# dog-qiuqiu/Yolo-FastestV2

Measured on NVIDIA B200. Metric: images/sec 352x352 fwd+decode+NMS, higher is better.
Workload: dtype f32

## Files before the change

yolo-fastestv2_b200/csrc/eng3.cuh:

```cuda
#pragma once
#include "common.cuh"
#include "tc.cuh"

namespace yfv2 {
namespace eng3 {

using namespace tc;

struct BPipe {
    uint64_t empty[2];
    uint64_t dfull;
    uint32_t arrivals[2];
};
struct BGrp {
    uint32_t tcol, tlane;
    BPipe* pipe;
    uint32_t chunk;
    uint32_t dparity;
    int gtid;
};

__device__ __forceinline__ uint32_t atom_inc_acq_rel(uint32_t* addr) {
    uint32_t old;
    asm volatile("atom.acq_rel.cta.shared::cta.add.u32 %0, [%1], 1;" : "=r"(old) : "r"(smem_u32(addr)) : "memory");
    return old;
}
__device__ __forceinline__ void publish_async() { asm volatile("fence.proxy.async.shared::cta;" ::: "memory"); }
__device__ __forceinline__ void tmem_ld16v(uint32_t taddr, float* v) {
    uint32_t r[16];
    asm volatile("tcgen05.ld.sync.aligned.32x32b.x16.b32 {%0, %1, %2, %3, %4, %5, %6, %7, %8, %9, %10, %11, %12, %13, %14, %15}, [%16];"
                 : "=r"(r[0]), "=r"(r[1]), "=r"(r[2]), "=r"(r[3]), "=r"(r[4]), "=r"(r[5]), "=r"(r[6]), "=r"(r[7]), "=r"(r[8]),
                   "=r"(r[9]), "=r"(r[10]), "=r"(r[11]), "=r"(r[12]), "=r"(r[13]), "=r"(r[14]), "=r"(r[15])
                 : "r"(taddr) : "memory");
#pragma unroll
    for (int i = 0; i < 16; ++i) v[i] = __uint_as_float(r[i]);
}


template <int NB>
__device__ __forceinline__ void st_acquire(BGrp& g) {
    const uint32_t buf = g.chunk % NB, use = g.chunk / NB;
    if (use > 0) mbar_wait(&g.pipe->empty[buf], (use - 1) & 1u);
    fence_after_sync();
}
template <int KC, int NB>
__device__ __forceinline__ void st_store(const BGrp& g, const float* a) {
    const uint32_t col = g.tlane + (g.chunk % NB) * (2 * KC);
#pragma unroll
    for (int j = 0; j < KC; j += 8) {
        uint32_t hi[8], lo[8];
#pragma unroll
        for (int i = 0; i < 8; ++i) {
            hi[i] = __float_as_uint(a[j + i]) & 0xFFFFE000u;
            lo[i] = __float_as_uint(a[j + i] - __uint_as_float(hi[i]));
        }
        tmem_st8(col + j, hi);
        tmem_st8(col + KC + j, lo);
    }
}
template <int KP, int NP, int KC, int NB>
__device__ __forceinline__ void st_hand_off(BGrp& g, int c, uint32_t b_hi, uint32_t b_lo, uint32_t dcol, bool last) {
    wait_st();
    fence_before_sync();
    __syncwarp();
    if ((threadIdx.x & 31) == 0) {
        const uint32_t buf = g.chunk % NB;
        const uint32_t old = atom_inc_acq_rel(&g.pipe->arrivals[buf]);
        if ((old & 3u) == 3u) {
            fence_after_sync();
            constexpr uint32_t idesc = make_idesc_tf32(128, NP);
            constexpr uint32_t LBO = 128, SBO = (KP / 4) * 128;
            const uint32_t a_hi = g.tcol + buf * (2 * KC), a_lo = a_hi + KC, d = g.tcol + dcol;
#pragma unroll
            for (int s = 0; s < KC / 8; ++s) {
                const int ks = c * (KC / 8) + s;
                const uint64_t bh = make_b_desc(b_hi + ks * 256, LBO, SBO);
                const uint64_t bl = make_b_desc(b_lo + ks * 256, LBO, SBO);
                mma_tf32_ts(d, a_lo + 8 * s, bh, idesc, ks > 0 ? 1u : 0u);
                mma_tf32_ts(d, a_hi + 8 * s, bl, idesc, 1u);
                mma_tf32_ts(d, a_hi + 8 * s, bh, idesc, 1u);
            }
            mma_commit(&g.pipe->empty[buf]);
            if (last) mma_commit(&g.pipe->dfull);
        }
    }
    __syncwarp();
    ++g.chunk;
}
__device__ __forceinline__ void st_wait_d(BGrp& g) {
    mbar_wait(&g.pipe->dfull, g.dparity);
    g.dparity ^= 1u;
    fence_after_sync();
}

}
}
```

yolo-fastestv2_b200/csrc/k_blk.cu:

```cuda
#include <cstdlib>

#include "eng3.cuh"

namespace yfv2 {
namespace {

using namespace tc;
using namespace eng3;

constexpr int kMaxChain = 7;
constexpr int kMaxK = 48;

template <int KC, int NB>
__device__ __forceinline__ void acquire_buf(BGrp& g) {
    const uint32_t buf = g.chunk % NB, use = g.chunk / NB;
    if (use > 0) mbar_wait(&g.pipe->empty[buf], (use - 1) & 1u);
    fence_after_sync();
}
template <int KC, int NB, int KCS = KC>
__device__ __forceinline__ void store_a(const BGrp& g, int tile, const float* a, int koff = 0) {
    const uint32_t col = g.tlane + (g.chunk % NB) * (4 * KC) + tile * (2 * KC) + koff;
#pragma unroll
    for (int j = 0; j < KCS; j += 8) {
        uint32_t hi[8], lo[8];
#pragma unroll
        for (int i = 0; i < 8; ++i) {
            hi[i] = __float_as_uint(a[j + i]) & 0xFFFFE000u;
            lo[i] = __float_as_uint(a[j + i] - __uint_as_float(hi[i]));
        }
        tmem_st8(col + j, hi);
        tmem_st8(col + KC + j, lo);
    }
}
template <int KP, int NP, int KC, int NB, int SIB = 1>
__device__ __forceinline__ void hand_off(BGrp& g, int c, uint32_t b_hi, uint32_t b_lo) {
    wait_st();
    fence_before_sync();
    __syncwarp();
    if ((threadIdx.x & 31) == 0) {
        const uint32_t buf = g.chunk % NB;
        const uint32_t old = atom_inc_acq_rel(&g.pipe->arrivals[buf]);
        if ((old & (4u * SIB - 1u)) == 4u * SIB - 1u) {
            fence_after_sync();
            constexpr uint32_t idesc = make_idesc_tf32(128, NP);
            constexpr uint32_t LBO = 128, SBO = (KP / 4) * 128;
#pragma unroll
            for (int t = 0; t < 2; ++t) {
                const uint32_t a_hi = g.tcol + buf * (4 * KC) + t * (2 * KC), a_lo = a_hi + KC;
                const uint32_t d = g.tcol + NB * 4 * KC + t * NP;
#pragma unroll
                for (int s = 0; s < KC / 8; ++s) {
                    const int ks = c * (KC / 8) + s;
                    const uint64_t bh = make_b_desc(b_hi + ks * 256, LBO, SBO);
                    const uint64_t bl = make_b_desc(b_lo + ks * 256, LBO, SBO);
                    mma_tf32_ts(d, a_lo + 8 * s, bh, idesc, ks > 0 ? 1u : 0u);
                    mma_tf32_ts(d, a_hi + 8 * s, bl, idesc, 1u);
                    mma_tf32_ts(d, a_hi + 8 * s, bh, idesc, 1u);
                }
            }
            mma_commit(&g.pipe->empty[buf]);
            if (c == KP / KC - 1) mma_commit(&g.pipe->dfull);
        }
    }
    __syncwarp();
    ++g.chunk;
}
template <int KC, int NB>
__device__ __forceinline__ void wait_d(BGrp& g) {
    mbar_wait(&g.pipe->dfull, g.dparity);
    g.dparity ^= 1u;
    fence_after_sync();
}
template <int NP, int KC, int NB>
__device__ __forceinline__ void load_d(const BGrp& g, int tile, float* d) {
#pragma unroll
    for (int n0 = 0; n0 < NP; n0 += 16) tmem_ld16v(g.tlane + NB * 4 * KC + tile * NP + n0, d + n0);
    wait_ld();
}

struct S1cArgs {
    Planes P;
    const float* w1[kMaxChain];
    const float* w2[kMaxChain];
    const float* wdw[kMaxChain];
    uint32_t in_off[kMaxChain][kMaxK];
    uint32_t out_off[kMaxChain][kMaxK];
    int nblk;
    int N, TR, bandsPerImg;
    int wbufs;
};

template <int K, int NP>
struct S1Smem {
    static constexpr int WFL = 2 * NP * K + 2 * NP;
    static constexpr int WSET = 2 * WFL + K * 12;
};
__host__ __device__ constexpr int t_half_floats(int TR, int W) { return ((TR + 3) / 2) * W + 2; }

template <int K, int NP, int G, int KC, int NB, int SIB = 1>
__global__ void __launch_bounds__(G * 128 * SIB, 1)
s1c_kernel(const __grid_constant__ S1cArgs p) {
    pdl_trigger();
    constexpr int KP = K;
    constexpr int COLS = NB * 4 * KC + 2 * NP;
    constexpr int KCS = KC / SIB, NT = G * 128 * SIB;
    static_assert(G * COLS <= 512 && K % KC == 0 && KCS % 8 == 0 && NP % 16 == 0 && K <= kMaxK && (SIB == 1 || SIB == 2), "shape");
    using L = S1Smem<K, NP>;
    extern __shared__ __align__(128) float smem[];
    __shared__ __align__(8) BPipe pipes[G];
    __shared__ __align__(8) uint64_t wbar[2];
    __shared__ uint32_t tmem_slot;
    float* sW = smem;
    float* T = sW + (size_t)p.wbufs * L::WSET;
    const int H = p.P.H, W = p.P.W;
    const int TH = t_half_floats(p.TR, W);
    const int TP = 2 * TH;
    const int warp = threadIdx.x >> 5;
    const int items = p.N * p.bandsPerImg;
    const int my_items = ((int)blockIdx.x < items) ? (items - 1 - (int)blockIdx.x) / (int)gridDim.x + 1 : 0;
    const int total_sets = p.nblk > 1 ? my_items * p.nblk : min(my_items, 1);

    auto load_wset = [&](int seq) {
        const int b = seq % p.nblk, buf = seq % p.wbufs;
        float* dst = sW + (size_t)buf * L::WSET;
        mbar_expect_tx(&wbar[buf], (uint32_t)(L::WSET * sizeof(float)));
        bulk_g2s(dst, p.w1[b], L::WFL * sizeof(float), &wbar[buf]);
        bulk_g2s(dst + L::WFL, p.w2[b], L::WFL * sizeof(float), &wbar[buf]);
        bulk_g2s(dst + 2 * L::WFL, p.wdw[b], K * 12 * sizeof(float), &wbar[buf]);
    };

    if (threadIdx.x == 32) {
        mbar_init(&wbar[0], 1); mbar_init(&wbar[1], 1);
        for (int i = 0; i < G; ++i) {
            mbar_init(&pipes[i].empty[0], 1); mbar_init(&pipes[i].empty[1], 1); mbar_init(&pipes[i].dfull, 1);
            pipes[i].arrivals[0] = 0; pipes[i].arrivals[1] = 0;
        }
        fence_mbar_init();
        if (total_sets > 0) load_wset(0);
        if (total_sets > 1 && p.wbufs > 1) load_wset(1);
    }
    if (warp == 0) tmem_alloc(&tmem_slot, 512);
    for (int i = threadIdx.x; i < K * TP; i += NT) T[i] = 0.f;
    fence_before_sync();
    __syncthreads();
    fence_after_sync();
    BGrp g;
    const int grp = threadIdx.x / (128 * SIB);
    const int sub = SIB == 1 ? 0 : (warp >> 2) & 1;
    const int koff = sub * KCS;
    g.tcol = tmem_slot + grp * COLS;
    g.tlane = g.tcol + ((uint32_t)(32 * (warp & 3)) << 16);
    g.pipe = &pipes[grp];
    g.chunk = 0; g.dparity = 0;
    g.gtid = threadIdx.x & 127;
    pdl_wait();

    int seq = 0;
    for (int item = blockIdx.x; item < items; item += gridDim.x) {
        const int n = item / p.bandsPerImg;
        const int r0 = (item - n * p.bandsPerImg) * p.TR;
        const int rows = min(p.TR, H - r0);
        float* const img = p.P.base + (long long)n * p.P.sN + p.P.org;
        const int tr_lo = r0 == 0 ? 1 : 0, tr_hi = (r0 + rows == H) ? rows : rows + 1;
        if (p.bandsPerImg > 1) {
            if (r0 == 0) for (int i = threadIdx.x; i < K * W; i += NT) { const int k = i / W; T[k * TP + 1 + (i - k * W)] = 0.f; }
            if (r0 + rows == H) {
                const int tr = rows + 1;
                const int o = (tr & 1) * TH + 1 + (tr >> 1) * W;
                for (int i = threadIdx.x; i < K * W; i += NT) { const int k = i / W; T[k * TP + o + (i - k * W)] = 0.f; }
            }
            __syncthreads();
        }
        for (int b = 0; b < p.nblk; ++b) {
            const int wb = seq % p.wbufs;
            const float* sB1 = sW + (size_t)wb * L::WSET;
            const float* sB2 = sB1 + L::WFL;
            const float* sDW = sB2 + L::WFL;
            mbar_wait(&wbar[wb], (uint32_t)(seq / p.wbufs) & 1u);
            const uint32_t b1_hi = smem_u32(sB1), b1_lo = smem_u32(sB1 + NP * KP);
            const uint32_t b2_hi = smem_u32(sB2), b2_lo = smem_u32(sB2 + NP * KP);
            const float* aff1 = sB1 + 2 * NP * KP;
            const float* aff2 = sB2 + 2 * NP * KP;
            const uint32_t* ioff = p.in_off[b];
            const uint32_t* ooff = p.out_off[b];
            const int i_lo = (tr_lo + 1) >> 1, i_hi = (tr_hi + 1) >> 1;
            const int nbp = (i_hi - i_lo + 1) * W;
            for (int tile = grp; tile * 128 < nbp; tile += G) {
                const int q = tile * 128 + g.gtid;
                const bool inb = q < nbp;
                const int qc = inb ? q : 0;
                const int ii = qc / W, x = qc - ii * W;
                const int i = i_lo + ii;
                const int tr0 = 2 * i - 1, tr1 = 2 * i;
                const bool v0 = inb && tr0 >= tr_lo, v1 = inb && tr1 <= tr_hi;
                const int gr0 = r0 - 1 + (tr0 >= tr_lo ? tr0 : tr1), gr1 = r0 - 1 + (tr1 <= tr_hi ? tr1 : tr0);
                const float* ip0 = img + gr0 * p.P.Ws + x;
                const float* ip1 = img + gr1 * p.P.Ws + x;
                float v[2][2 * KCS];
#pragma unroll
                for (int j = 0; j < KCS; ++j) { v[0][j] = __ldcg(ip0 + ioff[koff + j]); v[0][KCS + j] = __ldcg(ip1 + ioff[koff + j]); }
#pragma unroll
                for (int c = 0; c < K / KC; ++c) {
                    if (c + 1 < K / KC) {
#pragma unroll
                        for (int j = 0; j < KCS; ++j) {
                            v[(c + 1) & 1][j] = __ldcg(ip0 + ioff[(c + 1) * KC + koff + j]);
                            v[(c + 1) & 1][KCS + j] = __ldcg(ip1 + ioff[(c + 1) * KC + koff + j]);
                        }
                    }
                    acquire_buf<KC, NB>(g);
                    store_a<KC, NB, KCS>(g, 0, v[c & 1], koff);
                    store_a<KC, NB, KCS>(g, 1, v[c & 1] + KCS, koff);
                    hand_off<KP, NP, KC, NB, SIB>(g, c, b1_hi, b1_lo);
                }
                wait_d<KC, NB>(g);
                float* te = T + 1 + i * W + x;
                float* to = T + TH + 1 + (i - 1) * W + x;
#pragma unroll
                for (int t = 0; t < 2; ++t) {
                    if (SIB == 2 && t != sub) continue;
                    float d[NP];
                    load_d<NP, KC, NB>(g, t, d);
                    if (t == 0 ? v0 : v1) {
                        float* tp = t == 0 ? to : te;
#pragma unroll
                        for (int n4 = 0; n4 < K; n4 += 4) {
                            const float4 sc = *reinterpret_cast<const float4*>(aff1 + n4);
                            const float4 sh = *reinterpret_cast<const float4*>(aff1 + NP + n4);
                            tp[(n4 + 0) * TP] = fmaxf(fmaf(d[n4 + 0], sc.x, sh.x), 0.f);
                            tp[(n4 + 1) * TP] = fmaxf(fmaf(d[n4 + 1], sc.y, sh.y), 0.f);
                            tp[(n4 + 2) * TP] = fmaxf(fmaf(d[n4 + 2], sc.z, sh.z), 0.f);
                            tp[(n4 + 3) * TP] = fmaxf(fmaf(d[n4 + 3], sc.w, sh.w), 0.f);
                        }
                    }
                }
            }
            __syncthreads();
            const int ncp = ((rows + 1) >> 1) * W;
            for (int tile = grp; tile * 128 < ncp; tile += G) {
                const int q = tile * 128 + g.gtid;
                const bool inb = q < ncp;
                const int qc = inb ? q : 0;
                const int j = qc / W, ox = qc - j * W;
                const bool v0 = inb, v1 = inb && 2 * j + 1 < rows;
                const float mL = ox > 0 ? 1.f : 0.f, mR = ox < W - 1 ? 1.f : 0.f;
                const float* te = T + qc;
                const float* to = te + TH;
#pragma unroll 1
                for (int c = 0; c < K / KC; ++c) {
                    float a0[KCS], a1[KCS];
                    const float* e = te + (c * KC + koff) * TP;
                    const float* o = to + (c * KC + koff) * TP;
                    const float* wk = sDW + (c * KC + koff) * 12;
#pragma unroll
                    for (int jj = 0; jj < KCS; ++jj) {
                        const float4 wa = *reinterpret_cast<const float4*>(wk);
                        const float4 wb4 = *reinterpret_cast<const float4*>(wk + 4);
                        const float4 wc = *reinterpret_cast<const float4*>(wk + 8);
                        const float r0l = e[0], r0c = e[1], r0r = e[2];
                        const float r1l = o[0], r1c = o[1], r1r = o[2];
                        const float r2l = e[W], r2c = e[W + 1], r2r = e[W + 2];
                        const float r3l = o[W], r3c = o[W + 1], r3r = o[W + 2];
                        float cl0 = wa.x * r0l; cl0 = fmaf(wa.w, r1l, cl0); cl0 = fmaf(wb4.z, r2l, cl0);
                        float cc0 = wa.y * r0c; cc0 = fmaf(wb4.x, r1c, cc0); cc0 = fmaf(wb4.w, r2c, cc0);
                        float cr0 = wa.z * r0r; cr0 = fmaf(wb4.y, r1r, cr0); cr0 = fmaf(wc.x, r2r, cr0);
                        float cl1 = wa.x * r1l; cl1 = fmaf(wa.w, r2l, cl1); cl1 = fmaf(wb4.z, r3l, cl1);
                        float cc1 = wa.y * r1c; cc1 = fmaf(wb4.x, r2c, cc1); cc1 = fmaf(wb4.w, r3c, cc1);
                        float cr1 = wa.z * r1r; cr1 = fmaf(wb4.y, r2r, cr1); cr1 = fmaf(wc.x, r3r, cr1);
                        const float d0 = fmaf(mR, cr0, fmaf(mL, cl0, cc0));
                        const float d1 = fmaf(mR, cr1, fmaf(mL, cl1, cc1));
                        a0[jj] = fmaf(d0, wc.y, wc.z);
                        a1[jj] = fmaf(d1, wc.y, wc.z);
                        e += TP; o += TP; wk += 12;
                    }
                    acquire_buf<KC, NB>(g);
                    store_a<KC, NB, KCS>(g, 0, a0, koff);
                    store_a<KC, NB, KCS>(g, 1, a1, koff);
                    hand_off<KP, NP, KC, NB, SIB>(g, c, b2_hi, b2_lo);
                }
                wait_d<KC, NB>(g);
                float* op = img + (r0 + 2 * j) * p.P.Ws + ox;
#pragma unroll
                for (int t = 0; t < 2; ++t) {
                    if (SIB == 2 && t != sub) continue;
                    float d[NP];
                    load_d<NP, KC, NB>(g, t, d);
                    if (t == 0 ? v0 : v1) {
                        float* o2 = op + t * p.P.Ws;
#pragma unroll
                        for (int n4 = 0; n4 < K; n4 += 4) {
                            const float4 sc = *reinterpret_cast<const float4*>(aff2 + n4);
                            const float4 sh = *reinterpret_cast<const float4*>(aff2 + NP + n4);
                            o2[ooff[n4 + 0]] = fmaxf(fmaf(d[n4 + 0], sc.x, sh.x), 0.f);
                            o2[ooff[n4 + 1]] = fmaxf(fmaf(d[n4 + 1], sc.y, sh.y), 0.f);
                            o2[ooff[n4 + 2]] = fmaxf(fmaf(d[n4 + 2], sc.z, sh.z), 0.f);
                            o2[ooff[n4 + 3]] = fmaxf(fmaf(d[n4 + 3], sc.w, sh.w), 0.f);
                        }
                    }
                }
            }
            __syncthreads();
            if (p.nblk > 1) {
                if (threadIdx.x == 32 && seq + p.wbufs < total_sets) {
                    publish_async();
                    load_wset(seq + p.wbufs);
                }
                ++seq;
            }
        }
    }
    fence_before_sync();
    __syncthreads();
    if (warp == 0) tmem_dealloc(tmem_slot, 512);
}

template <int S>
__device__ __forceinline__ float dw3(const float* __restrict__ r0, const float* __restrict__ r1, const float* __restrict__ r2,
                                     const float* __restrict__ wk) {
    const float4 wa = *reinterpret_cast<const float4*>(wk);
    const float4 wb = *reinterpret_cast<const float4*>(wk + 4);
    const float4 wc = *reinterpret_cast<const float4*>(wk + 8);
    float p0 = wa.x * r0[0]; p0 = fmaf(wa.y, r0[1], p0); p0 = fmaf(wa.z, r0[2], p0);
    float p1 = wa.w * r1[0]; p1 = fmaf(wb.x, r1[1], p1); p1 = fmaf(wb.y, r1[2], p1);
    float p2 = wb.z * r2[0]; p2 = fmaf(wb.w, r2[1], p2); p2 = fmaf(wc.x, r2[2], p2);
    const float d = (p0 + p1) + p2;
    return fmaf(d, wc.y, wc.z);
}

__device__ __forceinline__ float dw3_s2_shfl(const float* __restrict__ t, int WS, const float* __restrict__ wk, bool nb_ok) {
    const float4 wa = *reinterpret_cast<const float4*>(wk);
    const float4 wb = *reinterpret_cast<const float4*>(wk + 4);
    const float4 wc = *reinterpret_cast<const float4*>(wk + 8);
    float2 v[3];
    float c2[3];
#pragma unroll
    for (int r = 0; r < 3; ++r) {
        v[r] = *reinterpret_cast<const float2*>(t + r * WS);
        c2[r] = __shfl_down_sync(0xffffffffu, v[r].x, 1);
        if (!nb_ok) c2[r] = t[r * WS + 2];
    }
    float p0 = wa.x * v[0].x; p0 = fmaf(wa.y, v[0].y, p0); p0 = fmaf(wa.z, c2[0], p0);
    float p1 = wa.w * v[1].x; p1 = fmaf(wb.x, v[1].y, p1); p1 = fmaf(wb.y, c2[1], p1);
    float p2 = wb.z * v[2].x; p2 = fmaf(wb.w, v[2].y, p2); p2 = fmaf(wc.x, c2[2], p2);
    const float d = (p0 + p1) + p2;
    return fmaf(d, wc.y, wc.z);
}

struct S2cArgs {
    Planes in, out;
    uint32_t in_off[kMaxK];
    uint32_t out_off[2 * kMaxK];
    const float* wp; const float* w1; const float* w2;
    const float* wdwp; const float* wdwm;
    int N, TR, bandsPerImg;
};

template <int K, int NP, int G, int KC, int NB>
__global__ void __launch_bounds__(G * 128 + 32, 1)
s2c_kernel(const __grid_constant__ S2cArgs p) {
    pdl_trigger();
    constexpr int KP = K, NCH = K / KC;
    constexpr int COLS = NB * 2 * KC + NP, DCOL = NB * 2 * KC;
    static_assert(G * COLS <= 512 && K % KC == 0 && KC % 8 == 0 && NP % 16 == 0 && K <= kMaxK, "shape");
    constexpr int WFL = 2 * NP * KP + 2 * NP;
    extern __shared__ __align__(128) float smem[];
    __shared__ __align__(8) BPipe pipes[G];
    __shared__ __align__(8) uint64_t wbar, xfull[2], xfree[2];
    __shared__ uint32_t tmem_slot;
    float* sBp = smem;
    float* sB1 = sBp + WFL;
    float* sB2 = sB1 + WFL;
    float* sDWp = sB2 + WFL;
    float* sDWm = sDWp + K * 12;
    float* Xb = sDWm + K * 12;
    const int Hin = p.in.H, Win = p.in.W, WS = p.in.Ws, pin = p.in.pad;
    const int Hout = p.out.H, Wout = p.out.W;
    const int XR = 2 * p.TR + 1;
    const int RS = XR * WS;
    const int XBUF = K * RS;
    const int warp = threadIdx.x >> 5;
    const int items = p.N * p.bandsPerImg;
    const int my_items = ((int)blockIdx.x < items) ? (items - 1 - (int)blockIdx.x) / (int)gridDim.x + 1 : 0;

    if (threadIdx.x == 0) {
        mbar_init(&wbar, 1);
        for (int i = 0; i < 2; ++i) { mbar_init(&xfull[i], 1); mbar_init(&xfree[i], G * 4); }
        for (int i = 0; i < G; ++i) {
            mbar_init(&pipes[i].empty[0], 1); mbar_init(&pipes[i].empty[1], 1); mbar_init(&pipes[i].dfull, 1);
            pipes[i].arrivals[0] = 0; pipes[i].arrivals[1] = 0;
        }
        fence_mbar_init();
        mbar_expect_tx(&wbar, (uint32_t)((3 * WFL + 2 * K * 12) * sizeof(float)));
        bulk_g2s(sBp, p.wp, WFL * sizeof(float), &wbar);
        bulk_g2s(sB1, p.w1, WFL * sizeof(float), &wbar);
        bulk_g2s(sB2, p.w2, WFL * sizeof(float), &wbar);
        bulk_g2s(sDWp, p.wdwp, K * 12 * sizeof(float), &wbar);
        bulk_g2s(sDWm, p.wdwm, K * 12 * sizeof(float), &wbar);
    }
    if (warp == 0) tmem_alloc(&tmem_slot, 512);
    fence_before_sync();
    __syncthreads();
    fence_after_sync();
    pdl_wait();

    auto item_geom = [&](int it, int& n, int& r0, int& rows) {
        const int item = (int)blockIdx.x + it * (int)gridDim.x;
        n = item / p.bandsPerImg;
        r0 = (item - n * p.bandsPerImg) * p.TR;
        rows = min(p.TR, Hout - r0);
    };

    if (warp == G * 4) {
        const int lane = threadIdx.x & 31;
        for (int it = 0; it < my_items; ++it) {
            const int buf = it & 1;
            int n, r0, rows;
            item_geom(it, n, r0, rows);
            const int nrows = 2 * rows + 1;
            if (it >= 2) mbar_wait(&xfree[buf], (uint32_t)((it >> 1) - 1) & 1u);
            publish_async();
            if (lane == 0) mbar_expect_tx(&xfull[buf], (uint32_t)(K * nrows * WS * sizeof(float)));
            __syncwarp();
            const float* src0 = p.in.base + (long long)n * p.in.sN + (long long)(2 * r0 - 1 + pin) * WS;
            for (int k = lane; k < K; k += 32)
                bulk_g2s(Xb + (size_t)buf * XBUF + (size_t)k * RS, src0 + p.in_off[k], (uint32_t)(nrows * WS * sizeof(float)), &xfull[buf]);
        }
    } else {
        BGrp g;
        const int grp = threadIdx.x >> 7;
        g.tcol = tmem_slot + grp * COLS;
        g.tlane = g.tcol + ((uint32_t)(32 * (warp & 3)) << 16);
        g.pipe = &pipes[grp];
        g.chunk = 0; g.dparity = 0;
        g.gtid = threadIdx.x & 127;
        const uint32_t bp_hi = smem_u32(sBp), bp_lo = smem_u32(sBp + NP * KP);
        const uint32_t b1_hi = smem_u32(sB1), b1_lo = smem_u32(sB1 + NP * KP);
        const uint32_t b2_hi = smem_u32(sB2), b2_lo = smem_u32(sB2 + NP * KP);
        const float* affp = sBp + 2 * NP * KP;
        const float* aff1 = sB1 + 2 * NP * KP;
        const float* aff2 = sB2 + 2 * NP * KP;
        mbar_wait(&wbar, 0);

        auto dw_tile = [&](const float* X, int n, int r0, int rows, int tile, const float* sDW, uint32_t b_hi, uint32_t b_lo,
                           const float* aff, const uint32_t* ooff) {
            const int npix = rows * Wout;
            const int q = tile * 128 + g.gtid;
            const bool valid = q < npix;
            const int qc = valid ? q : 0;
            const int orow = qc / Wout, ox = qc - orow * Wout;
            const float* w0 = X + (2 * orow) * WS + 2 * ox + (pin - 1);
            const bool aligned = (pin & 1) != 0;
            const bool nb_ok = ox + 1 < Wout && (threadIdx.x & 31) != 31;
#pragma unroll 1
            for (int c = 0; c < NCH; ++c) {
                float a[KC];
                const float* t = w0 + c * KC * RS;
                const float* wk = sDW + c * KC * 12;
                if (aligned) {
#pragma unroll
                    for (int j = 0; j < KC; ++j) { a[j] = dw3_s2_shfl(t, WS, wk, nb_ok); t += RS; wk += 12; }
                } else {
#pragma unroll
                    for (int j = 0; j < KC; ++j) { a[j] = dw3<2>(t, t + WS, t + 2 * WS, wk); t += RS; wk += 12; }
                }
                st_acquire<NB>(g);
                st_store<KC, NB>(g, a);
                st_hand_off<KP, NP, KC, NB>(g, c, b_hi, b_lo, DCOL, c == NCH - 1);
            }
            st_wait_d(g);
            float* op = p.out.base + (long long)n * p.out.sN + p.out.org + (r0 + orow) * p.out.Ws + ox;
#pragma unroll
            for (int n0 = 0; n0 < NP; n0 += 16) {
                if (n0 >= K) break;
                float d[16];
                tmem_ld16v(g.tlane + DCOL + n0, d);
                wait_ld();
                if (valid) {
#pragma unroll
                    for (int j = 0; j < 16; ++j)
                        if (n0 + j < K) op[ooff[n0 + j]] = fmaxf(fmaf(d[j], aff[n0 + j], aff[NP + n0 + j]), 0.f);
                }
            }
        };
        auto proj_tiles = [&](int it, int first, int step) {
            int n, r0, rows;
            item_geom(it, n, r0, rows);
            const float* X = Xb + (size_t)(it & 1) * XBUF;
            for (int tile = first; tile * 128 < rows * Wout; tile += step)
                dw_tile(X, n, r0, rows, tile, sDWp, bp_hi, bp_lo, affp, p.out_off);
        };

        if (my_items > 0) {
            mbar_wait(&xfull[0], 0);
            proj_tiles(0, grp, G);
            group_bar(1, G * 128);
        }
        for (int it = 0; it < my_items; ++it) {
            int n, r0, rows;
            item_geom(it, n, r0, rows);
            float* X = Xb + (size_t)(it & 1) * XBUF;
            const int gr0 = 2 * r0 - 1, nrows = 2 * rows + 1;
            const int gr_lo = max(gr0, 0), gr_hi = min(gr0 + nrows - 1, Hin - 1);
            const int npos = (gr_hi - gr_lo + 1) * Win;
            for (int tile = grp; tile * 128 < npos; tile += G) {
                const int q = tile * 128 + g.gtid;
                const bool valid = q < npos;
                const int qc = valid ? q : 0;
                const int rr = qc / Win, x = qc - rr * Win;
                float* tpos = X + (gr_lo + rr - gr0) * WS + pin + x;
#pragma unroll
                for (int c = 0; c < NCH; ++c) {
                    float a[KC];
#pragma unroll
                    for (int j = 0; j < KC; ++j) a[j] = tpos[(c * KC + j) * RS];
                    st_acquire<NB>(g);
                    st_store<KC, NB>(g, a);
                    st_hand_off<KP, NP, KC, NB>(g, c, b1_hi, b1_lo, DCOL, c == NCH - 1);
                }
                st_wait_d(g);
#pragma unroll
                for (int n0 = 0; n0 < NP; n0 += 16) {
                    if (n0 >= K) break;
                    float d[16];
                    tmem_ld16v(g.tlane + DCOL + n0, d);
                    wait_ld();
                    if (valid) {
#pragma unroll
                        for (int j = 0; j < 16; ++j)
                            if (n0 + j < K) tpos[(n0 + j) * RS] = fmaxf(fmaf(d[j], aff1[n0 + j], aff1[NP + n0 + j]), 0.f);
                    }
                }
            }
            group_bar(1, G * 128);
            const int mt = (rows * Wout + 127) / 128;
            const bool more = it + 1 < my_items;
            if (more) mbar_wait(&xfull[(it + 1) & 1], (uint32_t)((it + 1) >> 1) & 1u);
            for (int job = grp; job < mt; job += G)
                dw_tile(X, n, r0, rows, job, sDWm, b2_hi, b2_lo, aff2, p.out_off + K);
            if (more) proj_tiles(it + 1, ((grp - mt) % G + G) % G, G);
            group_bar(1, G * 128);
            if ((threadIdx.x & 31) == 0) mbar_arrive(&xfree[it & 1]);
        }
    }
    fence_before_sync();
    __syncthreads();
    if (warp == 0) tmem_dealloc(tmem_slot, 512);
}

constexpr int kPwMaxK = 288;
struct Pw3Args {
    Planes A, B, out;
    uint32_t in_off[kPwMaxK];
    uint32_t out_off[96];
    const float* wpack;
    int N, nout;
};

template <int KA, int KB, int SHA, int NP, int G, bool RELU, int KC = 16, int SIB = 1>
__global__ void __launch_bounds__(G * 128 * SIB, 1)
pw3_kernel(const __grid_constant__ Pw3Args p) {
    pdl_trigger();
    constexpr int KP = KA + KB, NB = 2, NCH = KP / KC, KCS = KC / SIB;
    constexpr int COLS = NB * 2 * KC + NP;
    static_assert(G * COLS <= 512 && KP % (2 * KC) == 0 && KA % KC == 0 && NP % 16 == 0 && KP <= kPwMaxK && KCS % 8 == 0 && (SIB == 1 || SIB == 2), "shape");
    extern __shared__ __align__(128) float smem[];
    __shared__ __align__(8) BPipe pipes[G];
    __shared__ __align__(8) uint64_t wbar;
    __shared__ uint32_t tmem_slot;
    float* sB = smem;
    constexpr int WFL = 2 * NP * KP + 2 * NP;
    const int warp = threadIdx.x >> 5;
    if (threadIdx.x == 32) {
        mbar_init(&wbar, 1);
        for (int i = 0; i < G; ++i) {
            mbar_init(&pipes[i].empty[0], 1); mbar_init(&pipes[i].empty[1], 1); mbar_init(&pipes[i].dfull, 1);
            pipes[i].arrivals[0] = 0; pipes[i].arrivals[1] = 0;
        }
        fence_mbar_init();
        mbar_expect_tx(&wbar, (uint32_t)(WFL * sizeof(float)));
        constexpr uint32_t kPiece = 32768;
        for (uint32_t o = 0; o < WFL * sizeof(float); o += kPiece)
            bulk_g2s(reinterpret_cast<char*>(sB) + o, reinterpret_cast<const char*>(p.wpack) + o,
                     min(kPiece, (uint32_t)(WFL * sizeof(float)) - o), &wbar);
    }
    if (warp == 0) tmem_alloc(&tmem_slot, 512);
    fence_before_sync();
    __syncthreads();
    fence_after_sync();
    BGrp g;
    const int grp = threadIdx.x / (128 * SIB);
    const int sub = SIB == 1 ? 0 : (warp >> 2) & 1;
    const int koff = sub * KCS;
    g.tcol = tmem_slot + grp * COLS;
    g.tlane = g.tcol + ((uint32_t)(32 * (warp & 3)) << 16);
    g.pipe = &pipes[grp];
    g.chunk = 0; g.dparity = 0;
    g.gtid = threadIdx.x & 127;
    const uint32_t b_hi = smem_u32(sB), b_lo = smem_u32(sB + NP * KP);
    const float* aff = sB + 2 * NP * KP;
    const int HW = p.out.H * p.out.W, W = p.out.W;
    const long long total = (long long)p.N * HW;
    const int ntiles = (int)((total + 127) / 128);
    constexpr int NBLK = NP / 16, H0 = (NBLK + 1) / 2;
    const int n_lo = SIB == 1 ? 0 : (sub ? H0 * 16 : 0), n_hi = SIB == 1 ? NP : (sub ? NP : H0 * 16);
    pdl_wait();
    mbar_wait(&wbar, 0);
    for (int tile = blockIdx.x * G + grp; tile < ntiles; tile += gridDim.x * G) {
        const long long pos = (long long)tile * 128 + g.gtid;
        const bool valid = pos < total;
        const long long pc = valid ? pos : 0;
        const int n = (int)(pc / HW);
        const int px = (int)(pc - (long long)n * HW);
        const int y = px / W, x = px - y * W;
        const float* baseA = p.A.base + (long long)n * p.A.sN + p.A.org + (y >> SHA) * p.A.Ws + (x >> SHA);
        const float* baseB = p.B.base + (long long)n * p.B.sN + p.B.org + y * p.B.Ws + x;
        float v[2][KCS];
        auto load = [&](int c, float* dst) {
            const float* base = (c * KC < KA) ? baseA : baseB;
#pragma unroll
            for (int j = 0; j < KCS; ++j) dst[j] = __ldcg(base + p.in_off[c * KC + koff + j]);
        };
        auto store = [&](const float* a) {
            const uint32_t col = g.tlane + (g.chunk % NB) * (2 * KC) + koff;
#pragma unroll
            for (int j = 0; j < KCS; j += 8) {
                uint32_t hi[8], lo[8];
#pragma unroll
                for (int i = 0; i < 8; ++i) {
                    hi[i] = __float_as_uint(a[j + i]) & 0xFFFFE000u;
                    lo[i] = __float_as_uint(a[j + i] - __uint_as_float(hi[i]));
                }
                tmem_st8(col + j, hi);
                tmem_st8(col + KC + j, lo);
            }
        };
        auto hand_off = [&](int c, bool last) {
            wait_st();
            fence_before_sync();
            __syncwarp();
            if ((threadIdx.x & 31) == 0) {
                const uint32_t buf = g.chunk % NB;
                const uint32_t old = atom_inc_acq_rel(&g.pipe->arrivals[buf]);
                if ((old & (4u * SIB - 1u)) == 4u * SIB - 1u) {
                    fence_after_sync();
                    constexpr uint32_t idesc = make_idesc_tf32(128, NP);
                    constexpr uint32_t LBO = 128, SBO = (KP / 4) * 128;
                    const uint32_t a_hi = g.tcol + buf * (2 * KC), a_lo = a_hi + KC, d = g.tcol + NB * 2 * KC;
#pragma unroll
                    for (int s2 = 0; s2 < KC / 8; ++s2) {
                        const int ks = c * (KC / 8) + s2;
                        const uint64_t bh = make_b_desc(b_hi + ks * 256, LBO, SBO);
                        const uint64_t bl = make_b_desc(b_lo + ks * 256, LBO, SBO);
                        mma_tf32_ts(d, a_lo + 8 * s2, bh, idesc, ks > 0 ? 1u : 0u);
                        mma_tf32_ts(d, a_hi + 8 * s2, bl, idesc, 1u);
                        mma_tf32_ts(d, a_hi + 8 * s2, bh, idesc, 1u);
                    }
                    mma_commit(&g.pipe->empty[buf]);
                    if (last) mma_commit(&g.pipe->dfull);
                }
            }
            __syncwarp();
            ++g.chunk;
        };
        load(0, v[0]);
#pragma unroll 1
        for (int c = 0; c < NCH; c += 2) {
            load(c + 1, v[1]);
            st_acquire<NB>(g);
            store(v[0]);
            hand_off(c, false);
            if (c + 2 < NCH) load(c + 2, v[0]);
            st_acquire<NB>(g);
            store(v[1]);
            hand_off(c + 1, c + 2 == NCH);
        }
        st_wait_d(g);
        float* obase = p.out.base + (long long)n * p.out.sN + p.out.org + y * p.out.Ws + x;
#pragma unroll
        for (int n0 = 0; n0 < NP; n0 += 16) {
            if (n0 < n_lo || n0 >= n_hi) continue;
            float d[16];
            tmem_ld16v(g.tlane + NB * 2 * KC + n0, d);
            wait_ld();
            if (valid) {
#pragma unroll
                for (int j = 0; j < 16; ++j) {
                    const int nn = n0 + j;
                    if (nn < p.nout) {
                        float r = fmaf(d[j], aff[nn], aff[NP + nn]);
                        if (RELU) r = fmaxf(r, 0.f);
                        obase[p.out_off[nn]] = r;
                    }
                }
            }
        }
    }
    fence_before_sync();
    __syncthreads();
    if (warp == 0) tmem_dealloc(tmem_slot, 512);
}

template <typename Kern>
int blk_smem_attr(Kern kern, size_t bytes) {
    if (bytes > kSmemCap) { set_error("block kernel needs %zu bytes of shared memory", bytes); return YFV2_EUNSUPPORTED; }
    YFV2_CUDA(cudaFuncSetAttribute(kern, cudaFuncAttributeMaxDynamicSharedMemorySize, (int)bytes));
    return YFV2_OK;
}

constexpr size_t kBlkSmemBudget = kSmemCap - 1024;

struct S1Geom { int TR, bands, wbufs; size_t bytes; bool whole; };
S1Geom s1_geometry(int K, int H, int W, int nblk) {
    const int NP = tc_round(K, 16);
    const size_t wset = (size_t)2 * (2 * NP * K + 2 * NP) + K * 12;
    auto need = [&](int tr, int wbufs) { return (wbufs * wset + (size_t)K * 2 * t_half_floats(tr, W)) * sizeof(float); };
    S1Geom g{};
    if (need(H, 1) <= kBlkSmemBudget) {
        g.whole = true; g.TR = H; g.bands = 1;
        g.wbufs = (nblk > 1 && need(H, 2) <= kBlkSmemBudget) ? 2 : 1;
        g.bytes = need(H, g.wbufs);
        return g;
    }
    g.whole = false; g.wbufs = 1;
    for (int nb = 2; nb <= H; ++nb) {
        const int tr = ((H + nb - 1) / nb + 1) & ~1;
        if (need(tr, 1) <= kBlkSmemBudget) { g.TR = tr; g.bands = (H + tr - 1) / tr; g.bytes = need(tr, 1); return g; }
    }
    g.TR = 0;
    return g;
}

}

bool blk_s1_chainable(int K, int H, int W) { return K <= kMaxK && s1_geometry(K, H, W, 2).whole; }

#define TRYB(x) do { int rc__ = (x); if (rc__) return rc__; } while (0)

int blk_launch_s1(int K, const Planes& P, int nblk, const ChanTab* tin, const ChanTab* tout, const float* const* w1,
                  const float* const* wdw, const float* const* w2, int N, cudaStream_t s, int* done) {
    if (K != 24 && K != 48) { set_error("blk_launch_s1: unsupported K=%d", K); return YFV2_EUNSUPPORTED; }
    if (nblk > kMaxChain) nblk = kMaxChain;
    S1Geom geo = s1_geometry(K, P.H, P.W, nblk);
    if (geo.TR <= 0) { set_error("blk_launch_s1: a %dx%d map does not fit in shared memory", P.H, P.W); return YFV2_EUNSUPPORTED; }
    if (!geo.whole) nblk = 1;
    S1cArgs a{};
    a.P = P; a.nblk = nblk; a.N = N; a.TR = geo.TR; a.bandsPerImg = geo.bands; a.wbufs = geo.wbufs;
    for (int b = 0; b < nblk; ++b) {
        a.w1[b] = w1[b]; a.w2[b] = w2[b]; a.wdw[b] = wdw[b];
        for (int k = 0; k < K; ++k) {
            a.in_off[b][k] = (uint32_t)((long long)tin[b].c[k] * P.sC);
            a.out_off[b][k] = (uint32_t)((long long)tout[b].c[k] * P.sC);
        }
    }
    const int items = N * geo.bands;
    auto run = [&](auto kern, int threads) -> int {
        TRYB(blk_smem_attr(kern, geo.bytes));
        YFV2_CUDA(launch_k(kern, min(items, sm_count()), threads, geo.bytes, s, pdl_take(), a));
        YFV2_LAUNCH_CHECK();
        return YFV2_OK;
    };
    *done = nblk;
    static const bool no_sib = getenv("YFV2_S1_NOSIB") != nullptr;
    if (K == 24) return run(s1c_kernel<24, 32, 4, 8, 2>, 4 * 128);
    if (no_sib) return run(s1c_kernel<48, 48, 2, 16, 2>, 2 * 128);
    return run(s1c_kernel<48, 48, 2, 16, 2, 2>, 2 * 256);
}

int blk_launch_s2(int K, const Planes& in, const Planes& out, const ChanTab& tin, const ChanTab& tout, const float* wdwp, const float* wp,
                  const float* w1, const float* wdwm, const float* w2, int N, cudaStream_t s) {
    if (K != 24 && K != 48) { set_error("blk_launch_s2: unsupported K=%d", K); return YFV2_EUNSUPPORTED; }
    S2cArgs a{};
    a.in = in; a.out = out; a.wp = wp; a.w1 = w1; a.w2 = w2; a.wdwp = wdwp; a.wdwm = wdwm; a.N = N;
    for (int k = 0; k < K; ++k) a.in_off[k] = (uint32_t)((long long)tin.c[k] * in.sC);
    for (int k = 0; k < 2 * K; ++k) a.out_off[k] = (uint32_t)((long long)tout.c[k] * out.sC);
    const int NP = tc_round(K, 16);
    const size_t wfl = (size_t)3 * (2 * NP * K + 2 * NP) + 2 * K * 12;
    auto bytes = [&](int tr) { return (wfl + (size_t)2 * K * (2 * tr + 1) * in.Ws) * sizeof(float); };
    int TR = out.H;
    while (TR > 1 && bytes(TR) > kBlkSmemBudget) --TR;
    if (bytes(TR) > kBlkSmemBudget) { set_error("blk_launch_s2: a %dx%d input does not fit in shared memory", in.H, in.W); return YFV2_EUNSUPPORTED; }
    const int bands = (out.H + TR - 1) / TR;
    TR = (out.H + bands - 1) / bands;
    a.TR = TR; a.bandsPerImg = (out.H + TR - 1) / TR;
    const int items = N * a.bandsPerImg;
    auto run = [&](auto kern, int G) -> int {
        TRYB(blk_smem_attr(kern, bytes(TR)));
        YFV2_CUDA(launch_k(kern, min(items, sm_count()), G * 128 + 32, bytes(TR), s, pdl_take(), a));
        YFV2_LAUNCH_CHECK();
        return YFV2_OK;
    };
    if (K == 24) return run(s2c_kernel<24, 32, 4, 24, 1>, 4);
    return run(s2c_kernel<48, 48, 4, 16, 2>, 4);
}

int blk_launch_pw(int kind, const Planes& A, const ChanTab& ta, const Planes& B, const ChanTab& tb, const Planes& out, const ChanTab& tout,
                  const float* wpack, int N, cudaStream_t s) {
    Pw3Args a{};
    a.A = A; a.B = B; a.out = out; a.wpack = wpack; a.N = N;
    const long long total = (long long)N * out.H * out.W;
    const int ntiles = (int)((total + 127) / 128);
    auto run = [&](auto kern, int KA, int KB, int NP, int G, int nout, int sib = 1) -> int {
        a.nout = nout;
        for (int k = 0; k < KA; ++k) a.in_off[k] = (uint32_t)((long long)ta.c[k] * A.sC);
        for (int k = 0; k < KB; ++k) a.in_off[KA + k] = (uint32_t)((long long)tb.c[k] * B.sC);
        for (int k = 0; k < nout; ++k) a.out_off[k] = (uint32_t)((long long)tout.c[k] * out.sC);
        const size_t bytes = (size_t)(2 * NP * (KA + KB) + 2 * NP) * sizeof(float);
        TRYB(blk_smem_attr(kern, bytes));
        YFV2_CUDA(launch_k(kern, min((ntiles + G - 1) / G, sm_count()), G * 128 * sib, bytes, s, pdl_take(), a));
        YFV2_LAUNCH_CHECK();
        return YFV2_OK;
    };
    static const int pw_sib = getenv("YFV2_PW_SIB") ? atoi(getenv("YFV2_PW_SIB")) : 1;
    if (pw_sib == 1) {
        if (kind == 0) return run(pw3_kernel<96, 0, 0, 96, 3, true, 16, 2>, 96, 0, 96, 3, 96, 2);
        if (kind == 1) return run(pw3_kernel<192, 0, 0, 80, 3, true, 16, 2>, 192, 0, 80, 3, 72, 2);
        if (kind == 2) return run(pw3_kernel<192, 96, 1, 80, 3, true, 16, 2>, 192, 96, 80, 3, 72, 2);
    } else if (pw_sib == 2) {
        if (kind == 0) return run(pw3_kernel<96, 0, 0, 96, 2, true, 16, 2>, 96, 0, 96, 2, 96, 2);
        if (kind == 1) return run(pw3_kernel<192, 0, 0, 80, 2, true, 16, 2>, 192, 0, 80, 2, 72, 2);
        if (kind == 2) return run(pw3_kernel<192, 96, 1, 80, 2, true, 16, 2>, 192, 96, 80, 2, 72, 2);
    }
    if (kind == 0) return run(pw3_kernel<96, 0, 0, 96, 3, true>, 96, 0, 96, 3, 96);
    if (kind == 1) return run(pw3_kernel<192, 0, 0, 80, 3, true>, 192, 0, 80, 3, 72);
    if (kind == 2) return run(pw3_kernel<192, 96, 1, 80, 3, true>, 192, 96, 80, 3, 72);
    if (kind == 3) return run(pw3_kernel<48, 0, 0, 48, 4, true, 8>, 48, 0, 48, 4, 48);
    set_error("blk_launch_pw: unknown kind %d", kind);
    return YFV2_EUNSUPPORTED;
}

}
```

Measured before the change: 161,000.

## Pair warpgroups to split channel chunks in stride-2 depthwise tiles

New measurement: 163,700 (median of 6 runs). 1.02x the previous value.

```diff
diff --git a/yolo-fastestv2_b200/csrc/eng3.cuh b/yolo-fastestv2_b200/csrc/eng3.cuh
--- a/yolo-fastestv2_b200/csrc/eng3.cuh
+++ b/yolo-fastestv2_b200/csrc/eng3.cuh
@@ -43,11 +43,11 @@
     if (use > 0) mbar_wait(&g.pipe->empty[buf], (use - 1) & 1u);
     fence_after_sync();
 }
-template <int KC, int NB>
-__device__ __forceinline__ void st_store(const BGrp& g, const float* a) {
-    const uint32_t col = g.tlane + (g.chunk % NB) * (2 * KC);
+template <int KC, int NB, int KCS = KC>
+__device__ __forceinline__ void st_store(const BGrp& g, const float* a, int koff = 0) {
+    const uint32_t col = g.tlane + (g.chunk % NB) * (2 * KC) + koff;
 #pragma unroll
-    for (int j = 0; j < KC; j += 8) {
+    for (int j = 0; j < KCS; j += 8) {
         uint32_t hi[8], lo[8];
 #pragma unroll
         for (int i = 0; i < 8; ++i) {
@@ -58,15 +58,16 @@
         tmem_st8(col + KC + j, lo);
     }
 }
-template <int KP, int NP, int KC, int NB>
+template <int KP, int NP, int KC, int NB, int NW = 4>
 __device__ __forceinline__ void st_hand_off(BGrp& g, int c, uint32_t b_hi, uint32_t b_lo, uint32_t dcol, bool last) {
+    static_assert(NW == 4 || NW == 8, "arrival count");
     wait_st();
     fence_before_sync();
     __syncwarp();
     if ((threadIdx.x & 31) == 0) {
         const uint32_t buf = g.chunk % NB;
         const uint32_t old = atom_inc_acq_rel(&g.pipe->arrivals[buf]);
-        if ((old & 3u) == 3u) {
+        if ((old & (NW - 1u)) == NW - 1u) {
             fence_after_sync();
             constexpr uint32_t idesc = make_idesc_tf32(128, NP);
             constexpr uint32_t LBO = 128, SBO = (KP / 4) * 128;
diff --git a/yolo-fastestv2_b200/csrc/k_blk.cu b/yolo-fastestv2_b200/csrc/k_blk.cu
--- a/yolo-fastestv2_b200/csrc/k_blk.cu
+++ b/yolo-fastestv2_b200/csrc/k_blk.cu
@@ -1,4 +1,5 @@
 #include <cstdlib>
+#include <type_traits>
 
 #include "eng3.cuh"
 
@@ -345,6 +346,23 @@
     const float d = (p0 + p1) + p2;
     return fmaf(d, wc.y, wc.z);
 }
+__device__ __forceinline__ float dw3_s2_ld(const float* __restrict__ t, int WS, const float* __restrict__ wk) {
+    const float4 wa = *reinterpret_cast<const float4*>(wk);
+    const float4 wb = *reinterpret_cast<const float4*>(wk + 4);
+    const float4 wc = *reinterpret_cast<const float4*>(wk + 8);
+    float2 v[3];
+    float c2[3];
+#pragma unroll
+    for (int r = 0; r < 3; ++r) {
+        v[r] = *reinterpret_cast<const float2*>(t + r * WS);
+        c2[r] = t[r * WS + 2];
+    }
+    float p0 = wa.x * v[0].x; p0 = fmaf(wa.y, v[0].y, p0); p0 = fmaf(wa.z, c2[0], p0);
+    float p1 = wa.w * v[1].x; p1 = fmaf(wb.x, v[1].y, p1); p1 = fmaf(wb.y, c2[1], p1);
+    float p2 = wb.z * v[2].x; p2 = fmaf(wb.w, v[2].y, p2); p2 = fmaf(wc.x, c2[2], p2);
+    const float d = (p0 + p1) + p2;
+    return fmaf(d, wc.y, wc.z);
+}
 
 struct S2cArgs {
     Planes in, out;
@@ -355,16 +373,19 @@
     int N, TR, bandsPerImg;
 };
 
-template <int K, int NP, int G, int KC, int NB>
+template <int K, int NP, int G, int KC, int NB, bool R2 = false>
 __global__ void __launch_bounds__(G * 128 + 32, 1)
 s2c_kernel(const __grid_constant__ S2cArgs p) {
     pdl_trigger();
     constexpr int KP = K, NCH = K / KC;
     constexpr int COLS = NB * 2 * KC + NP, DCOL = NB * 2 * KC;
+    constexpr int MG = (!R2 && KC % 16 == 0 && NP % 16 == 0 && G % 2 == 0) ? 2 : 1;
+    constexpr int KCS = KC / MG, NS = G / MG;
     static_assert(G * COLS <= 512 && K % KC == 0 && KC % 8 == 0 && NP % 16 == 0 && K <= kMaxK, "shape");
     constexpr int WFL = 2 * NP * KP + 2 * NP;
     extern __shared__ __align__(128) float smem[];
     __shared__ __align__(8) BPipe pipes[G];
+    __shared__ __align__(8) BPipe ppipes[MG == 2 ? NS : 1];
     __shared__ __align__(8) uint64_t wbar, xfull[2], xfree[2];
     __shared__ uint32_t tmem_slot;
     float* sBp = smem;
@@ -389,6 +410,12 @@
             mbar_init(&pipes[i].empty[0], 1); mbar_init(&pipes[i].empty[1], 1); mbar_init(&pipes[i].dfull, 1);
             pipes[i].arrivals[0] = 0; pipes[i].arrivals[1] = 0;
         }
+        if (MG == 2) {
+            for (int i = 0; i < NS; ++i) {
+                mbar_init(&ppipes[i].empty[0], 1); mbar_init(&ppipes[i].empty[1], 1); mbar_init(&ppipes[i].dfull, 1);
+                ppipes[i].arrivals[0] = 0; ppipes[i].arrivals[1] = 0;
+            }
+        }
         fence_mbar_init();
         mbar_expect_tx(&wbar, (uint32_t)((3 * WFL + 2 * K * 12) * sizeof(float)));
         bulk_g2s(sBp, p.wp, WFL * sizeof(float), &wbar);
@@ -433,6 +460,16 @@
         g.pipe = &pipes[grp];
         g.chunk = 0; g.dparity = 0;
         g.gtid = threadIdx.x & 127;
+        BGrp gp = g;
+        if (MG == 2) {
+            gp.tcol = tmem_slot + (grp & ~1) * COLS;
+            gp.tlane = gp.tcol + ((uint32_t)(32 * (warp & 3)) << 16);
+            gp.pipe = &ppipes[MG == 2 ? grp / MG : 0];
+        }
+        BGrp& gm = MG == 2 ? gp : g;
+        const int slot = grp / MG;
+        const int sub = MG == 2 ? (grp & 1) : 0;
+        const int koff = sub * KCS;
         const uint32_t bp_hi = smem_u32(sBp), bp_lo = smem_u32(sBp + NP * KP);
         const uint32_t b1_hi = smem_u32(sB1), b1_lo = smem_u32(sB1 + NP * KP);
         const uint32_t b2_hi = smem_u32(sB2), b2_lo = smem_u32(sB2 + NP * KP);
@@ -440,11 +477,16 @@
         const float* aff1 = sB1 + 2 * NP * KP;
         const float* aff2 = sB2 + 2 * NP * KP;
         mbar_wait(&wbar, 0);
+        auto phase_bar = [&]() {
+            if (MG == 2) fence_before_sync();
+            group_bar(1, G * 128);
+            if (MG == 2) fence_after_sync();
+        };
 
         auto dw_tile = [&](const float* X, int n, int r0, int rows, int tile, const float* sDW, uint32_t b_hi, uint32_t b_lo,
                            const float* aff, const uint32_t* ooff) {
             const int npix = rows * Wout;
-            const int q = tile * 128 + g.gtid;
+            const int q = tile * 128 + gm.gtid;
             const bool valid = q < npix;
             const int qc = valid ? q : 0;
             const int orow = qc / Wout, ox = qc - orow * Wout;
@@ -453,33 +495,60 @@
             const bool nb_ok = ox + 1 < Wout && (threadIdx.x & 31) != 31;
 #pragma unroll 1
             for (int c = 0; c < NCH; ++c) {
-                float a[KC];
-                const float* t = w0 + c * KC * RS;
-                const float* wk = sDW + c * KC * 12;
+                float a[KCS];
+                const float* t = w0 + (c * KC + koff) * RS;
+                const float* wk = sDW + (c * KC + koff) * 12;
                 if (aligned) {
 #pragma unroll
-                    for (int j = 0; j < KC; ++j) { a[j] = dw3_s2_shfl(t, WS, wk, nb_ok); t += RS; wk += 12; }
+                    for (int j = 0; j < KCS; ++j) {
+                        a[j] = R2 ? dw3_s2_shfl(t, WS, wk, nb_ok) : dw3_s2_ld(t, WS, wk);
+                        t += RS; wk += 12;
+                    }
                 } else {
 #pragma unroll
-                    for (int j = 0; j < KC; ++j) { a[j] = dw3<2>(t, t + WS, t + 2 * WS, wk); t += RS; wk += 12; }
-                }
-                st_acquire<NB>(g);
-                st_store<KC, NB>(g, a);
-                st_hand_off<KP, NP, KC, NB>(g, c, b_hi, b_lo, DCOL, c == NCH - 1);
-            }
-            st_wait_d(g);
+                    for (int j = 0; j < KCS; ++j) { a[j] = dw3<2>(t, t + WS, t + 2 * WS, wk); t += RS; wk += 12; }
+                }
+                st_acquire<NB>(gm);
+                st_store<KC, NB, KCS>(gm, a, koff);
+                st_hand_off<KP, NP, KC, NB, 4 * MG>(gm, c, b_hi, b_lo, DCOL, c == NCH - 1);
+            }
+            st_wait_d(gm);
             float* op = p.out.base + (long long)n * p.out.sN + p.out.org + (r0 + orow) * p.out.Ws + ox;
-#pragma unroll
-            for (int n0 = 0; n0 < NP; n0 += 16) {
-                if (n0 >= K) break;
-                float d[16];
-                tmem_ld16v(g.tlane + DCOL + n0, d);
-                wait_ld();
-                if (valid) {
-#pragma unroll
-                    for (int j = 0; j < 16; ++j)
-                        if (n0 + j < K) op[ooff[n0 + j]] = fmaxf(fmaf(d[j], aff[n0 + j], aff[NP + n0 + j]), 0.f);
-                }
+            if constexpr (MG == 1) {
+#pragma unroll
+                for (int n0 = 0; n0 < NP; n0 += 16) {
+                    if (n0 >= K) break;
+                    float d[16];
+                    tmem_ld16v(gm.tlane + DCOL + n0, d);
+                    wait_ld();
+                    if (valid) {
+#pragma unroll
+                        for (int j = 0; j < 16; ++j)
+                            if (n0 + j < K) op[ooff[n0 + j]] = fmaxf(fmaf(d[j], aff[n0 + j], aff[NP + n0 + j]), 0.f);
+                    }
+                }
+            } else {
+                auto drain = [&](auto base) {
+                    constexpr int B0 = decltype(base)::value, HALF = NP / 2;
+                    float d[HALF / 8][8];
+#pragma unroll
+                    for (int j = 0; j < HALF / 8; ++j) tmem_ld8(gm.tlane + DCOL + B0 + 8 * j, d[j]);
+                    wait_ld();
+                    if (valid) {
+#pragma unroll
+                        for (int j = 0; j < HALF; j += 4) {
+                            if (B0 + j >= K) break;
+                            const float4 sc = *reinterpret_cast<const float4*>(aff + B0 + j);
+                            const float4 sh = *reinterpret_cast<const float4*>(aff + NP + B0 + j);
+                            op[ooff[B0 + j + 0]] = fmaxf(fmaf(d[j / 8][j % 8 + 0], sc.x, sh.x), 0.f);
+                            op[ooff[B0 + j + 1]] = fmaxf(fmaf(d[j / 8][j % 8 + 1], sc.y, sh.y), 0.f);
+                            op[ooff[B0 + j + 2]] = fmaxf(fmaf(d[j / 8][j % 8 + 2], sc.z, sh.z), 0.f);
+                            op[ooff[B0 + j + 3]] = fmaxf(fmaf(d[j / 8][j % 8 + 3], sc.w, sh.w), 0.f);
+                        }
+                    }
+                };
+                if (sub == 0) drain(std::integral_constant<int, 0>());
+                else drain(std::integral_constant<int, NP / 2>());
             }
         };
         auto proj_tiles = [&](int it, int first, int step) {
@@ -492,8 +561,8 @@
 
         if (my_items > 0) {
             mbar_wait(&xfull[0], 0);
-            proj_tiles(0, grp, G);
-            group_bar(1, G * 128);
+            proj_tiles(0, slot, NS);
+            phase_bar();
         }
         for (int it = 0; it < my_items; ++it) {
             int n, r0, rows;
@@ -525,20 +594,33 @@
                     tmem_ld16v(g.tlane + DCOL + n0, d);
                     wait_ld();
                     if (valid) {
-#pragma unroll
-                        for (int j = 0; j < 16; ++j)
-                            if (n0 + j < K) tpos[(n0 + j) * RS] = fmaxf(fmaf(d[j], aff1[n0 + j], aff1[NP + n0 + j]), 0.f);
+                        if constexpr (R2) {
+#pragma unroll
+                            for (int j = 0; j < 16; ++j)
+                                if (n0 + j < K) tpos[(n0 + j) * RS] = fmaxf(fmaf(d[j], aff1[n0 + j], aff1[NP + n0 + j]), 0.f);
+                        } else {
+#pragma unroll
+                            for (int j = 0; j < 16; j += 4) {
+                                if (n0 + j >= K) break;
+                                const float4 sc = *reinterpret_cast<const float4*>(aff1 + n0 + j);
+                                const float4 sh = *reinterpret_cast<const float4*>(aff1 + NP + n0 + j);
+                                tpos[(n0 + j + 0) * RS] = fmaxf(fmaf(d[j + 0], sc.x, sh.x), 0.f);
+                                tpos[(n0 + j + 1) * RS] = fmaxf(fmaf(d[j + 1], sc.y, sh.y), 0.f);
+                                tpos[(n0 + j + 2) * RS] = fmaxf(fmaf(d[j + 2], sc.z, sh.z), 0.f);
+                                tpos[(n0 + j + 3) * RS] = fmaxf(fmaf(d[j + 3], sc.w, sh.w), 0.f);
+                            }
+                        }
                     }
                 }
             }
-            group_bar(1, G * 128);
+            phase_bar();
             const int mt = (rows * Wout + 127) / 128;
             const bool more = it + 1 < my_items;
             if (more) mbar_wait(&xfull[(it + 1) & 1], (uint32_t)((it + 1) >> 1) & 1u);
-            for (int job = grp; job < mt; job += G)
+            for (int job = slot; job < mt; job += NS)
                 dw_tile(X, n, r0, rows, job, sDWm, b2_hi, b2_lo, aff2, p.out_off + K);
-            if (more) proj_tiles(it + 1, ((grp - mt) % G + G) % G, G);
-            group_bar(1, G * 128);
+            if (more) proj_tiles(it + 1, ((slot - mt) % NS + NS) % NS, NS);
+            phase_bar();
             if ((threadIdx.x & 31) == 0) mbar_arrive(&xfree[it & 1]);
         }
     }
@@ -789,8 +871,9 @@
         YFV2_LAUNCH_CHECK();
         return YFV2_OK;
     };
-    if (K == 24) return run(s2c_kernel<24, 32, 4, 24, 1>, 4);
-    return run(s2c_kernel<48, 48, 4, 16, 2>, 4);
+    static const bool r2 = getenv("YFV2_S2C_R2") != nullptr;
+    if (K == 24) return r2 ? run(s2c_kernel<24, 32, 4, 24, 1, true>, 4) : run(s2c_kernel<24, 32, 4, 24, 1>, 4);
+    return r2 ? run(s2c_kernel<48, 48, 4, 16, 2, true>, 4) : run(s2c_kernel<48, 48, 4, 16, 2>, 4);
 }
 
 int blk_launch_pw(int kind, const Planes& A, const ChanTab& ta, const Planes& B, const ChanTab& tb, const Planes& out, const ChanTab& tout,
```
